# masnottuh/point-cloud-toolbox

Measured on AMD Instinct MI355X. Metric: points/sec curvature (1M-pt torus, k=50); HBM GB/s k-NN vs peak, higher is better.
Workload: dtype f64

## Files before the change

### point-cloud-toolbox_amd/csrc/pct_grid.hip

```cpp
#include "pct_internal.h"
#include "pct_grid_edge.h"

#include <math.h>
#include <stdlib.h>

namespace {

constexpr int kBlock = 256;

__device__ __forceinline__ float wave_min(float v) {
    for (int o = 32; o > 0; o >>= 1) v = fminf(v, __shfl_xor(v, o));
    return v;
}
__device__ __forceinline__ float wave_max(float v) {
    for (int o = 32; o > 0; o >>= 1) v = fmaxf(v, __shfl_xor(v, o));
    return v;
}

struct PackRed {
    int bb[6];
    int bad;
    int g_begin;
    double s[3], ss[3];
    unsigned long long cnt;
// ... 441 lines not shown
        }
        rank_of[i] = atomicAdd(&cell_oth[c], 1) | (int)0x80000000;
    }
}

__global__ __launch_bounds__(kBlock) void k_hist_raw(const float* __restrict__ xyz, int64_t n, pct_grid g, int q_begin, int q_end,
                                                     int* __restrict__ cell_of, int* __restrict__ rank_of,
                                                     int* __restrict__ cell_own, int* __restrict__ cell_oth, PackRed* __restrict__ parts) {
    const float sh[3] = {0.f, 0.f, 0.f};
    PackAcc acc;
    acc.init();
    const int64_t i = (int64_t)blockIdx.x * kBlock + threadIdx.x;
    if (i < n) {
        const float x = xyz[3 * i + 0], y = xyz[3 * i + 1], z = xyz[3 * i + 2];
        const bool ok = isfinite(x) && isfinite(y) && isfinite(z);
        acc.bad |= !ok;
        if (ok) acc.add(x, y, z, sh);
        const int cx = cell_coord(ok ? (double)x : g.ox, g.ox, g.inv_cell, g.nx);
        const int cy = cell_coord(ok ? (double)y : g.oy, g.oy, g.inv_cell, g.ny);
        const int cz = cell_coord(ok ? (double)z : g.oz, g.oz, g.inv_cell, g.nz);
        const int c = (cz * g.ny + cy) * g.nx + cx;
        cell_of[i] = c;
        if (i >= q_begin && i < q_end) rank_of[i] = atomicAdd(&cell_own[c], 1);
        else rank_of[i] = atomicAdd(&cell_oth[c], 1) | (int)0x80000000;
    }
    if (parts) acc.commit(parts + blockIdx.x);
}

__global__ __launch_bounds__(kBlock) void k_hist_agg(const float4* __restrict__ pts4, int64_t n, pct_grid g,
                                                     const float* __restrict__ own_want, float own_lo, float own_hi, int skip_outside,
                                                     int* __restrict__ cell_of, int* __restrict__ rank_of,
                                                     int* __restrict__ cell_own, int* __restrict__ cell_oth) {
    const int64_t i = (int64_t)blockIdx.x * kBlock + threadIdx.x;
    const int lane = threadIdx.x & 63;
    int key = -1;
    if (i < n) {
        const float4 p = pts4[i];
        bool inside = true;
        if (skip_outside) {
            const double fx = floor(((double)p.x - g.ox) * g.inv_cell), fy = floor(((double)p.y - g.oy) * g.inv_cell),
                         fz = floor(((double)p.z - g.oz) * g.inv_cell);
            inside = !(fx < 0 || fx >= g.nx || fy < 0 || fy >= g.ny || fz < 0 || fz >= g.nz);
        }
        if (inside) {
            const int cx = cell_coord((double)p.x, g.ox, g.inv_cell, g.nx);
            const int cy = cell_coord((double)p.y, g.oy, g.inv_cell, g.ny);
            const int cz = cell_coord((double)p.z, g.oz, g.inv_cell, g.nz);
            const int c = (cz * g.ny + cy) * g.nx + cx;
            const float w = own_want[__float_as_int(p.w)];
            const bool owned = w >= own_lo && w < own_hi;
            if (owned || !skip_outside || __builtin_nontemporal_load(&cell_oth[c]) <= 2048) key = 2 * c + (owned ? 1 : 0);
        }
    }
    int rank = 0;
    unsigned long long todo = __builtin_amdgcn_ballot_w64(key >= 0);
    while (todo) {
        const int leader = (int)__builtin_ctzll(todo);
        const int k0 = __builtin_amdgcn_readlane(key, leader);
        const unsigned long long same = __builtin_amdgcn_ballot_w64(key == k0);
        int base = 0;
        if (lane == leader) base = atomicAdd((k0 & 1) ? &cell_own[k0 >> 1] : &cell_oth[k0 >> 1], (int)__popcll(same));
        base = __builtin_amdgcn_readlane(base, leader);
        if (key == k0) rank = base + (int)__popcll(same & ((1ull << lane) - 1ull));
        todo &= ~same;
    }
    if (i < n) {
        cell_of[i] = key < 0 ? -1 : key >> 1;
        if (key >= 0) rank_of[i] = (key & 1) ? rank : (rank | (int)0x80000000);
    }
}

constexpr int kScanItems = 8;
constexpr int kScanTile = kBlock * kScanItems;

__device__ __forceinline__ int4 add3(int4 a, int4 b) { return make_int4(a.x + b.x, a.y + b.y, a.z + b.z, a.w + b.w); }

__device__ __forceinline__ int4 cell_counts(const int* __restrict__ own, const int* __restrict__ oth, int64_t c, int64_t ncell, int items_q) {
    if (c >= ncell) return make_int4(0, 0, 0, 0);
    const int o = own[c];
    const int t = o + (oth ? oth[c] : 0);
    return make_int4(t, (o + items_q - 1) / items_q, o, t > 0 ? 1 : 0);
}

__global__ __launch_bounds__(kBlock) void k_scan_sums(const int* __restrict__ own, const int* __restrict__ oth, int64_t ncell, int items_q,
                                                      int4* __restrict__ tmp, unsigned long long* __restrict__ sq_part) {
    __shared__ int4 sh[kBlock / 64];
    __shared__ unsigned long long shq[kBlock / 64];
    unsigned long long sq = 0;
    int64_t base = (int64_t)blockIdx.x * kScanTile + (int64_t)threadIdx.x * kScanItems;
    int4 v = make_int4(0, 0, 0, 0);
    for (int j = 0; j < kScanItems; ++j) {
        const int4 x = cell_counts(own, oth, base + j, ncell, items_q);
        v = add3(v, x);
        sq += (unsigned long long)x.z * (unsigned)x.x;
    }
    for (int o = 32; o > 0; o >>= 1) {
        v.x += __shfl_xor(v.x, o); v.y += __shfl_xor(v.y, o); v.z += __shfl_xor(v.z, o); v.w += __shfl_xor(v.w, o);
        sq += __shfl_xor(sq, o);
    }
    if ((threadIdx.x & 63) == 0) {
        sh[threadIdx.x >> 6] = v;
        shq[threadIdx.x >> 6] = sq;
    }
    __syncthreads();
    if (threadIdx.x == 0) {
        int4 t = make_int4(0, 0, 0, 0);
        unsigned long long q = 0;
        for (int i = 0; i < kBlock / 64; ++i) { t = add3(t, sh[i]); q += shq[i]; }
        tmp[blockIdx.x] = t;
        sq_part[blockIdx.x] = q;
    }
}

struct ScanTotals { unsigned long long sumsq; int4 tot; };

__global__ __launch_bounds__(1024) void k_scan_tiles(int4* __restrict__ tmp, int nblk, const unsigned long long* __restrict__ sq_part,
                                                      ScanTotals* __restrict__ host_copy, unsigned long long* __restrict__ zero8) {
    __shared__ int4 sh[1024];
    if (zero8 && threadIdx.x < 8) zero8[threadIdx.x] = 0ull;
    __shared__ int4 carry;
    __shared__ unsigned long long shq[16];
    {
        unsigned long long q = 0;
        for (int i = threadIdx.x; i < nblk; i += 1024) q += sq_part[i];
        for (int o = 32; o > 0; o >>= 1) q += __shfl_xor(q, o);
        if ((threadIdx.x & 63) == 0) shq[threadIdx.x >> 6] = q;
        __syncthreads();
        if (threadIdx.x == 0) { unsigned long long t = 0; for (int i = 0; i < 16; ++i) t += shq[i]; host_copy->sumsq = t; }
    }
    if (threadIdx.x == 0) carry = make_int4(0, 0, 0, 0);
    __syncthreads();
    for (int base = 0; base < nblk; base += 1024) {
        int i = base + threadIdx.x;
        int4 v = i < nblk ? tmp[i] : make_int4(0, 0, 0, 0);
        sh[threadIdx.x] = v;
        __syncthreads();
        for (int o = 1; o < 1024; o <<= 1) {
            int4 a = make_int4(0, 0, 0, 0);
            if ((int)threadIdx.x >= o) a = sh[threadIdx.x - o];
            __syncthreads();
            sh[threadIdx.x] = add3(sh[threadIdx.x], a);
            __syncthreads();
        }
        int4 incl = sh[threadIdx.x];
        int4 c = carry;
        if (i < nblk) tmp[i] = make_int4(c.x + incl.x - v.x, c.y + incl.y - v.y, c.z + incl.z - v.z, 0);
        __syncthreads();
        if (threadIdx.x == 1023) carry = add3(c, incl);
        __syncthreads();
    }
    if (threadIdx.x == 0) { tmp[nblk] = carry; host_copy->tot = carry; }
}

__global__ __launch_bounds__(kBlock) void k_scan_apply(const int* __restrict__ own, const int* __restrict__ oth, int64_t ncell, int items_q,
                                                       const int4* __restrict__ tmp, int* __restrict__ cell_start,
                                                       int* __restrict__ own_start, int2* __restrict__ items) {
    __shared__ int4 sh[kBlock];
    int64_t base = (int64_t)blockIdx.x * kScanTile + (int64_t)threadIdx.x * kScanItems;
    int4 x[kScanItems];
    int4 v = make_int4(0, 0, 0, 0);
    for (int j = 0; j < kScanItems; ++j) {
        x[j] = cell_counts(own, oth, base + j, ncell, items_q);
        v = add3(v, x[j]);
    }
    sh[threadIdx.x] = v;
    __syncthreads();
// ... 111 lines not shown
                const bool ok = isfinite(p[j].x) && isfinite(p[j].y) && isfinite(p[j].z);
                acc.bad |= !ok;
                if (ok) acc.add(p[j].x, p[j].y, p[j].z, sh);
            }
            atomicAdd(&s_cnt[bin_cell(p[j].x, p[j].y, p[j].z, g) >> shift], 1u);
        }
    }
    __syncthreads();
    for (int b = threadIdx.x; b < nb; b += kBinWide) mat[(size_t)blockIdx.x * nb + b] = s_cnt[b];
    if (parts) acc.commit<kBinWide / 64>(parts + blockIdx.x);
}

constexpr int kBinScanCols = 16, kBinScanGroups = 64, kBinScanPer = kBinMaxTiles / kBinScanGroups;
__global__ __launch_bounds__(kBinScanCols * kBinScanGroups) void k_bin_colscan(unsigned* __restrict__ mat, int ntiles, int nb, unsigned* __restrict__ tot) {
    __shared__ unsigned s[kBinScanGroups][kBinScanCols];
    const int lane = threadIdx.x % kBinScanCols, grp = threadIdx.x / kBinScanCols;
    const int col = blockIdx.x * kBinScanCols + lane;
    const int per = (ntiles + kBinScanGroups - 1) / kBinScanGroups;
    const int t0 = grp * per;
    unsigned v[kBinScanPer], sum = 0;
#pragma unroll
    for (int j = 0; j < kBinScanPer; ++j) {
        v[j] = (j < per && t0 + j < ntiles && col < nb) ? mat[(size_t)(t0 + j) * nb + col] : 0u;
        sum += v[j];
    }
    s[grp][lane] = sum;
    __syncthreads();
    unsigned run = 0;
    for (int q = 0; q < grp; ++q) run += s[q][lane];
    if (col >= nb) return;
#pragma unroll
    for (int j = 0; j < kBinScanPer; ++j) {
        if (j < per && t0 + j < ntiles) mat[(size_t)(t0 + j) * nb + col] = run;
        run += v[j];
    }
    if (grp == kBinScanGroups - 1) tot[col] = run;
}

__global__ __launch_bounds__(1024) void k_bin_plan(const unsigned* __restrict__ tot, int nb, int chunk, int* __restrict__ plan,
                                                   int4* __restrict__ items) {
    __shared__ int4 sh[1024];
    constexpr int per = kBinMaxBuckets / 1024;
    int4 v[per];
    int4 mine = make_int4(0, 0, 0, 0);
    for (int j = 0; j < per; ++j) {
        const int b = threadIdx.x * per + j;
        const int c = b < nb ? (int)tot[b] : 0;
        const int ni = b < nb ? max(1, (c + chunk - 1) / chunk) : 0;
        v[j] = make_int4(c, ni, ni > 1 ? ni : 0, ni > 1 ? 1 : 0);
        mine = add3(mine, v[j]);
    }
    sh[threadIdx.x] = mine;
    __syncthreads();
    for (int o = 1; o < 1024; o <<= 1) {
        int4 a = make_int4(0, 0, 0, 0);
        if ((int)threadIdx.x >= o) a = sh[threadIdx.x - o];
        __syncthreads();
        sh[threadIdx.x] = add3(sh[threadIdx.x], a);
        __syncthreads();
    }
    int4 run = make_int4(sh[threadIdx.x].x - mine.x, sh[threadIdx.x].y - mine.y, sh[threadIdx.x].z - mine.z, 0);
    int* bstart = plan + 16;
    for (int j = 0; j < per; ++j) {
        const int b = threadIdx.x * per + j;
        if (b < nb) {
            bstart[b] = run.x;
            for (int ch = 0; ch < v[j].y; ++ch)
                items[run.y + ch] = make_int4(b, run.x + ch * chunk, run.x + min(v[j].x, (ch + 1) * chunk), v[j].z ? run.z + ch : -1);
        }
        run = add3(run, v[j]);
    }
    if (threadIdx.x == 1023) {
        bstart[nb] = run.x;
        plan[0] = run.y;
        plan[1] = run.z;
        plan[2] = sh[1023].w;
    }
}

template <bool RAW>
__global__ __launch_bounds__(kBinWide) void k_bin_scatter(const float* __restrict__ xyz, const float4* __restrict__ pts4, int64_t n,
                                                           int tile_rows, pct_grid g, int shift, int nb, int chunk,
                                                           const unsigned* __restrict__ mat, const int* __restrict__ plan,
                                                           float4* __restrict__ rec, int* __restrict__ cell_own, int* __restrict__ cell_oth) {
    __shared__ unsigned s_cur[kBinMaxBuckets];
    const int* bstart = plan + 16;
    for (int b = threadIdx.x; b < nb; b += kBinWide) s_cur[b] = (unsigned)bstart[b] + mat[(size_t)blockIdx.x * nb + b];
    __syncthreads();
    const int64_t r0 = (int64_t)blockIdx.x * tile_rows, r1 = min(n, r0 + tile_rows);
    for (int64_t base = r0 + threadIdx.x; base < r1; base += 4 * kBinWide) {
        float4 p[4];
#pragma unroll
        for (int j = 0; j < 4; ++j)
            if (base + j * kBinWide < r1) p[j] = bin_load<RAW>(xyz, pts4, base + j * kBinWide);
#pragma unroll
        for (int j = 0; j < 4; ++j) {
            if (base + j * kBinWide >= r1) continue;
            const unsigned pos = atomicAdd(&s_cur[bin_cell(p[j].x, p[j].y, p[j].z, g) >> shift], 1u);
            if (pos < (unsigned)n) rec[pos] = p[j];
        }
    }
    if (plan[2] > 0) {
        for (int b = blockIdx.x; b < nb; b += gridDim.x) {
            if (bstart[b + 1] - bstart[b] <= chunk) continue;
            const int64_t c0 = (int64_t)b << shift, c1 = min(g.ncell, c0 + ((int64_t)1 << shift));
            for (int64_t c = c0 + threadIdx.x; c < c1; c += kBinWide) {
                cell_own[c] = 0;
                if (cell_oth) cell_oth[c] = 0;
            }
        }
    }
}

__global__ __launch_bounds__(kBinBlock) void k_bin_cells(const float4* __restrict__ rec, const int* __restrict__ plan,
                                                         const int4* __restrict__ items, pct_grid g, int shift, int q_begin, int q_end,
                                                         int* __restrict__ cell_own, int* __restrict__ cell_oth, int* __restrict__ base,
                                                         const PackRed* __restrict__ parts, int n_parts, PackRed* __restrict__ red,
                                                         PackRed* __restrict__ red_host) {
    extern __shared__ int s_c[];
    if (blockIdx.x == gridDim.x - 1) {
        if (parts) pack_fold<kBinBlock>(parts, n_parts, red, red_host, 0);
        return;
    }
    if ((int)blockIdx.x >= plan[0]) return;
    const int4 it = items[blockIdx.x];
    const int r0 = it.y, r1 = it.z, slot = it.w;
    const int cpb = 1 << shift, nc = cell_oth ? 2 * cpb : cpb;
    const int64_t c0 = (int64_t)it.x << shift;
    const int ncl = (int)min((int64_t)cpb, g.ncell - c0);
    for (int k = threadIdx.x; k < nc; k += kBinBlock) s_c[k] = 0;
    __syncthreads();
    for (int base = r0 + threadIdx.x; base < r1; base += 4 * kBinBlock) {
        float4 p[4];
#pragma unroll
        for (int j = 0; j < 4; ++j)
            if (base + j * kBinBlock < r1) p[j] = rec[base + j * kBinBlock];
#pragma unroll
        for (int j = 0; j < 4; ++j) {
            if (base + j * kBinBlock >= r1) continue;
            const int l = bin_cell(p[j].x, p[j].y, p[j].z, g) - (int)c0;
            const int idx = __float_as_int(p[j].w);
            const bool owned = !cell_oth || (idx >= q_begin && idx < q_end);
            if ((unsigned)l < (unsigned)cpb) atomicAdd(&s_c[(owned ? 0 : cpb) + l], 1);
        }
    }
    __syncthreads();
    for (int k = threadIdx.x; k < nc; k += kBinBlock) {
        const int l = k & (cpb - 1);
        if (l >= ncl) continue;
        int* arr = k < cpb ? cell_own : cell_oth;
        const int v = s_c[k];
        if (slot < 0) arr[c0 + l] = v;
        else base[(size_t)slot * nc + k] = v ? atomicAdd(&arr[c0 + l], v) : 0;
    }
}

__global__ __launch_bounds__(kBinBlock) void k_bin_place(const float4* __restrict__ rec, const int* __restrict__ plan,
                                                         const int4* __restrict__ items, pct_grid g, int shift, int q_begin, int q_end,
                                                         int64_t n, int64_t n_owned, const int* __restrict__ cell_start,
                                                         const int* __restrict__ cell_own, const int* __restrict__ cell_oth,
                                                         const int* __restrict__ own_start, const int* __restrict__ base,
                                                         float4* __restrict__ sorted4, int* __restrict__ row_of, int* __restrict__ owned_pos,
                                                         const double4* __restrict__ pts4d, double4* __restrict__ sorted4d) {
    extern __shared__ int s_cur[];
    if ((int)blockIdx.x >= plan[0]) return;
    const int4 it = items[blockIdx.x];
    const int r0 = it.y, r1 = it.z, slot = it.w;
    if (r0 >= r1) return;
    const int cpb = 1 << shift, nc = cell_oth ? 2 * cpb : cpb;
    const int64_t c0 = (int64_t)it.x << shift;
    const int ncl = (int)min((int64_t)cpb, g.ncell - c0);
    int* s_row = s_cur + nc;
    for (int k = threadIdx.x; k < nc; k += kBinBlock) {
        const int l = k & (cpb - 1);
        if (l >= ncl) continue;
        int s = cell_start[c0 + l];
        if (k >= cpb) s += cell_own[c0 + l];
        else if (cell_oth) s_row[l] = own_start[c0 + l] - s;
        if (slot >= 0) s += base[(size_t)slot * nc + k];
        s_cur[k] = s;
    }
    __syncthreads();
    for (int base = r0 + threadIdx.x; base < r1; base += 4 * kBinBlock) {
        float4 p[4];
#pragma unroll
        for (int j = 0; j < 4; ++j)
            if (base + j * kBinBlock < r1) p[j] = rec[base + j * kBinBlock];
#pragma unroll
        for (int j = 0; j < 4; ++j) {
            if (base + j * kBinBlock >= r1) continue;
            const int l = bin_cell(p[j].x, p[j].y, p[j].z, g) - (int)c0;
            const int idx = __float_as_int(p[j].w);
            const bool owned = !cell_oth || (idx >= q_begin && idx < q_end);
            if ((unsigned)l >= (unsigned)ncl) continue;
            const int pos = atomicAdd(&s_cur[(owned ? 0 : cpb) + l], 1);
            if ((unsigned)pos >= (unsigned)n) continue;
            sorted4[pos] = p[j];
            if (pts4d) sorted4d[pos] = pts4d[idx];
            if (owned) {
                const int row = cell_oth ? pos + s_row[l] : pos;
                if ((unsigned)row < (unsigned)n_owned && (unsigned)(idx - q_begin) < (unsigned)n_owned) {
                    owned_pos[row] = pos;
                    if (row_of) row_of[idx - q_begin] = row;
                }
            }
        }
    }
}

__global__ __launch_bounds__(256) void k_bin_row_of(const float4* __restrict__ sorted4, const int* __restrict__ owned_pos, int64_t n_owned,
                                                    int q_begin, int* __restrict__ row_of) {
    const int64_t row = (int64_t)blockIdx.x * 256 + threadIdx.x;
    if (row >= n_owned) return;
    const int idx = __float_as_int(sorted4[owned_pos[row]].w);
    if ((unsigned)(idx - q_begin) < (unsigned)n_owned) row_of[idx - q_begin] = (int)row;
}

__global__ __launch_bounds__(256) void k_gather_int(const int* __restrict__ map, int* __restrict__ io, int64_t n) {
    const int64_t i = (int64_t)blockIdx.x * 256 + threadIdx.x;
    if (i < n) io[i] = map[io[i]];
}

int grid_1d(int64_t n, int per_block, int cap) {
    int64_t b = (n + per_block - 1) / per_block;
    if (b < 1) b = 1;
    if (cap > 0 && b > cap) b = cap;
    return (int)b;
}

}

static PackRed* red_parts(pct_ctx* ctx) { return (PackRed*)((char*)ctx->red.p + 128); }
static_assert(sizeof(PackRed) <= sizeof(pct_pinned::pack_red) && alignof(PackRed) <= 128, "pct_pinned::pack_red holds a PackRed");
static_assert(sizeof(ScanTotals) <= sizeof(pct_pinned::scan_totals) && alignof(ScanTotals) <= 128, "pct_pinned::scan_totals holds a ScanTotals");
static PackRed* pin_red(pct_ctx* ctx) { return (PackRed*)ctx->pin->pack_red; }
static ScanTotals* pin_totals(pct_ctx* ctx) { return (ScanTotals*)ctx->pin->scan_totals; }

static int red_reset(pct_ctx* ctx, int n_parts, bool zero = true) {
    PCT_TRY(pct_reserve(ctx, &ctx->red, 128 + (size_t)n_parts * sizeof(PackRed)));
    if (zero) PCT_HIP(ctx, hipMemsetAsync(ctx->red.p, 0, 128, ctx->stream));
    return PCT_OK;
}

static int red_fold(pct_ctx* ctx, int n_parts, bool carry = true) {
    PCT_LAUNCH(k_pack_final, dim3(1), dim3(kBlock), 0, ctx->stream, (const PackRed*)red_parts(ctx), n_parts,
                       (PackRed*)ctx->red.p, pin_red(ctx), carry ? 1 : 0);
    PCT_HIP(ctx, hipGetLastError());
    return PCT_OK;
}

static int red_read(pct_ctx* ctx, int n_parts, PackRed* out, float* bbox, bool carry = true) {
    PCT_TRY(red_fold(ctx, n_parts, carry));
    PCT_HIP(ctx, hipStreamSynchronize(ctx->stream));
    memcpy(out, pin_red(ctx), sizeof(*out));
    for (int a = 0; a < 6; ++a) bbox[a] = order_float(out->bb[a]);
    return PCT_OK;
}

static int pack_all(pct_ctx* ctx, float* bbox, PackRed* red, bool defer = false, unsigned long long* begin_stamp = nullptr) {
    const int64_t n = ctx->n;
    PCT_TRY(pct_reserve(ctx, &ctx->pts4, (size_t)n * sizeof(float4)));
    const int nb = grid_1d(n, kBlock * 4, 512);
    PCT_TRY(red_reset(ctx, nb, false));
    PCT_LAUNCH(k_pack, dim3(nb), dim3(kBlock), 0, ctx->stream, ctx->xyz_view, n, (float4*)ctx->pts4.p, red_parts(ctx), begin_stamp);
    PCT_HIP(ctx, hipGetLastError());
    if (defer) {
        PCT_TRY(red_fold(ctx, nb, false));
    } else {
        PCT_TRY(red_read(ctx, nb, red, bbox, false));
        if (red->bad) return pct_fail(ctx, PCT_ERR_NONFINITE, "Non-finite values in input points");
// ... 244 lines not shown
        break;
    }
    s->raw = s->deferred_box = s->src == GridSource::CallerRows;
    s->from_base = s->src == GridSource::LevelBase;
    s->n = ctx->n_grid;
    s->g_begin = own_flag ? 0 : (int)ctx->g_begin;
    s->g_end = own_flag ? 0 : (int)(ctx->g_begin + n_owned);
    return PCT_OK;
}

enum class BoxCheck { Accept, Restart, NonFinite };
static BoxCheck check_deferred_box(pct_ctx* ctx, GridPoints* s) {
    s->deferred_box = false;
    memcpy(&s->red, pin_red(ctx), sizeof(s->red));
    if (s->red.bad) return BoxCheck::NonFinite;
    bool same = true;
    for (int ax = 0; ax < 3; ++ax) {
        const float lo = order_float(s->red.bb[ax]), hi = order_float(s->red.bb[3 + ax]);
        const float tol = 0.02f * (ctx->spec_raw[3 + ax] - ctx->spec_raw[ax]) + 1e-30f;
        same = same && fabsf(lo - ctx->spec_raw[ax]) <= tol && fabsf(hi - ctx->spec_raw[3 + ax]) <= tol;
    }
    return same ? BoxCheck::Accept : BoxCheck::Restart;
}

static void size_grid(const pct_ctx* ctx, bool sub_box, float* bbox, double a, pct_grid* g) {
    if (sub_box)
        for (int ax = 0; ax < 3; ++ax) {
            bbox[ax] = ctx->level_box[ax] - (float)(2.5 * a);
            bbox[3 + ax] = ctx->level_box[3 + ax] + (float)(2.5 * a);
        }
    g->ox = bbox[0]; g->oy = bbox[1]; g->oz = bbox[2];
    g->cell = a;
    g->inv_cell = 1.0 / a;
    double ex = (double)bbox[3] - bbox[0], ey = (double)bbox[4] - bbox[1], ez = (double)bbox[5] - bbox[2];
    if (!(ex >= 0)) ex = 0;
    if (!(ey >= 0)) ey = 0;
    if (!(ez >= 0)) ez = 0;
    const double dx = floor(ex * g->inv_cell) + 1, dy = floor(ey * g->inv_cell) + 1, dz = floor(ez * g->inv_cell) + 1;
    if (!(dx * dy * dz < 4.0e18) || !(dx < 2.0e9) || !(dy < 2.0e9) || !(dz < 2.0e9)) {
        g->nx = g->ny = g->nz = 1 << 30;
        g->ncell = (int64_t)1 << 62;
        return;
    }
    g->nx = (int32_t)dx;
    g->ny = (int32_t)dy;
    g->nz = (int32_t)dz;
    g->ncell = (int64_t)g->nx * g->ny * g->nz;
}

static int reserve_lists(pct_ctx* ctx, int64_t n, int64_t n_owned) {
    PCT_TRY(pct_reserve(ctx, &ctx->cell_of, (size_t)n * sizeof(int)));
    PCT_TRY(pct_reserve(ctx, &ctx->cell_fill, (size_t)n * sizeof(int)));
    PCT_TRY(pct_reserve(ctx, &ctx->sorted4, (size_t)n * sizeof(float4)));
    PCT_TRY(pct_reserve(ctx, &ctx->row_of, (size_t)((ctx->own_flag ? n : n_owned) + 1) * sizeof(int)));
    PCT_TRY(pct_reserve(ctx, &ctx->owned_pos, (size_t)n_owned * sizeof(int)));
    if (ctx->has_f64) PCT_TRY(pct_reserve(ctx, &ctx->sorted4d, (size_t)n * sizeof(double4)));
    return PCT_OK;
}

static EdgeSearch edge_search(const pct_ctx* ctx, const GridPoints& s, double target, double eps) {
    EdgeSearch es = {};
    es.target = target; es.n = s.n; es.eps = eps;
    es.ex = (double)s.bbox[3] - s.bbox[0]; es.ey = (double)s.bbox[4] - s.bbox[1]; es.ez = (double)s.bbox[5] - s.bbox[2];
    es.hint_edge = ctx->hint_edge; es.hint_guess = ctx->hint_guess; es.hint_target = ctx->hint_target;
    es.level_edge = ctx->level_edge;
    es.max_iter = es.level_edge > 0 ? 1 : ctx->level_mode ? 2 : 8;
    return es;
}

enum class GridBuild {
    Bin,
    AtomicRaw,
    AtomicBase,
    AtomicPacked,
};
static GridBuild choose_build(bool bin_allowed, const BinShape& bs, const GridPoints& s) {
    return bin_allowed && bs.ok ? GridBuild::Bin : s.raw ? GridBuild::AtomicRaw : s.from_base ? GridBuild::AtomicBase : GridBuild::AtomicPacked;
}

struct BinScratch {
    int* plan;
    unsigned* tot;
    int4* items;
    size_t lds;
};
static int bin_scratch(pct_ctx* ctx, const BinShape& bs, int64_t n, BinScratch* b) {
    PCT_TRY(pct_reserve(ctx, &ctx->bin_rec, (size_t)n * sizeof(float4)));
    PCT_TRY(pct_reserve(ctx, &ctx->bin_mat, (size_t)bs.ntiles * bs.nb * sizeof(unsigned)));
    const size_t plan_words = 16 + (size_t)(bs.nb + 1) + (size_t)bs.nb;
    const size_t items_at = (plan_words * sizeof(int) + 15) / 16 * 16;
    PCT_TRY(pct_reserve(ctx, &ctx->bin_plan, items_at + (size_t)bs.max_items * sizeof(int4)));
    PCT_TRY(pct_reserve(ctx, &ctx->bin_base, (size_t)bs.max_shared * (bs.cls << bs.shift) * sizeof(int)));
    b->plan = (int*)ctx->bin_plan.p;
    b->tot = (unsigned*)(b->plan + 16 + bs.nb + 1);
    b->items = (int4*)((char*)ctx->bin_plan.p + items_at);
    b->lds = (size_t)(bs.cls << bs.shift) * sizeof(int);
    return PCT_OK;
}

struct GridPass {
    GridBuild build;
    pct_grid g;
    BinShape bs;
    BinScratch bin;
    const float4* src;
    int64_t n_owned;
    bool sharded, sub_box;
};

template <bool RAW>
static void launch_bin_count(pct_ctx* ctx, int64_t n, const GridPass& p, PackRed* parts, unsigned long long* begin_stamp) {
    PCT_LAUNCH_T(k_bin_count<RAW>, dim3(p.bs.ntiles), dim3(kBinWide), 0, ctx->stream, ctx->xyz_view, p.src, n, p.bs.tile_rows, p.g, p.bs.shift,
                 p.bs.nb, (unsigned*)ctx->bin_mat.p, parts, begin_stamp);
}
template <bool RAW>
static void launch_bin_scatter(pct_ctx* ctx, int64_t n, const GridPass& p, int* cell_oth) {
    PCT_LAUNCH_T(k_bin_scatter<RAW>, dim3(p.bs.ntiles), dim3(kBinWide), 0, ctx->stream, ctx->xyz_view, p.src, n, p.bs.tile_rows, p.g, p.bs.shift,
                 p.bs.nb, p.bs.chunk, (const unsigned*)ctx->bin_mat.p, (const int*)p.bin.plan, (float4*)ctx->bin_rec.p, (int*)ctx->cell_own.p, cell_oth);
}

static int launch_count(pct_ctx* ctx, const GridPoints& s, GridPass& p, pct_call_clock* clock) {
    const pct_grid& g = p.g;
    const int64_t n = s.n;
    const float* own_flag = (const float*)ctx->own_flag;
    const bool bin = p.build == GridBuild::Bin;
    PCT_TRY(pct_reserve(ctx, &ctx->cell_own, (size_t)g.ncell * sizeof(int)));
    if (clock && !bin) PCT_HIP(ctx, clock->begin_event(ctx->stream));
    if (!bin) PCT_HIP(ctx, hipMemsetAsync(ctx->cell_own.p, 0, (size_t)g.ncell * sizeof(int), ctx->stream));
    if (p.sharded) {
        PCT_TRY(pct_reserve(ctx, &ctx->cell_oth, (size_t)g.ncell * sizeof(int)));
        if (!bin) PCT_HIP(ctx, hipMemsetAsync(ctx->cell_oth.p, 0, (size_t)g.ncell * sizeof(int), ctx->stream));
    }
    if (bin) PCT_TRY(bin_scratch(ctx, p.bs, n, &p.bin));
    int* cell_oth = p.sharded ? (int*)ctx->cell_oth.p : nullptr;
    PackRed* parts = s.deferred_box ? red_parts(ctx) : nullptr;
    const int nhb = grid_1d(n, kBlock, 0);
    if (bin) {
        const BinShape& bs = p.bs;
        unsigned long long* begin_stamp = clock ? clock->begin_word() : nullptr;
        s.raw ? launch_bin_count<true>(ctx, n, p, parts, begin_stamp) : launch_bin_count<false>(ctx, n, p, parts, begin_stamp);
        PCT_LAUNCH(k_bin_colscan, dim3((bs.nb + kBinScanCols - 1) / kBinScanCols), dim3(kBinScanCols * kBinScanGroups), 0, ctx->stream,
                   (unsigned*)ctx->bin_mat.p, bs.ntiles, bs.nb, p.bin.tot);
        PCT_LAUNCH(k_bin_plan, dim3(1), dim3(1024), 0, ctx->stream, (const unsigned*)p.bin.tot, bs.nb, bs.chunk, p.bin.plan, p.bin.items);
        s.raw ? launch_bin_scatter<true>(ctx, n, p, cell_oth) : launch_bin_scatter<false>(ctx, n, p, cell_oth);
        PCT_LAUNCH(k_bin_cells, dim3(bs.max_items + 1), dim3(kBinBlock), p.bin.lds, ctx->stream, (const float4*)ctx->bin_rec.p, (const int*)p.bin.plan,
                   (const int4*)p.bin.items, g, bs.shift, (int)ctx->q_begin, (int)ctx->q_end, (int*)ctx->cell_own.p, cell_oth,
                   (int*)ctx->bin_base.p, (const PackRed*)parts, bs.ntiles, (PackRed*)ctx->red.p, pin_red(ctx));
    } else if (p.build == GridBuild::AtomicRaw) {
        PCT_LAUNCH(k_hist_raw, dim3(nhb), dim3(kBlock), 0, ctx->stream, ctx->xyz_view, n, g, s.g_begin, s.g_end, (int*)ctx->cell_of.p,
                   (int*)ctx->cell_fill.p, (int*)ctx->cell_own.p, cell_oth, parts);
        if (parts) PCT_TRY(red_fold(ctx, nhb, false));
    } else if (p.build == GridBuild::AtomicBase) {
        PCT_LAUNCH(k_hist_agg, dim3(nhb), dim3(kBlock), 0, ctx->stream, p.src, n, g, own_flag, ctx->own_lo, ctx->own_hi, p.sub_box ? 1 : 0,
                   (int*)ctx->cell_of.p, (int*)ctx->cell_fill.p, (int*)ctx->cell_own.p, (int*)ctx->cell_oth.p);
    } else {
        PCT_LAUNCH(k_hist, dim3(nhb), dim3(kBlock), 0, ctx->stream, p.src, n, g, s.g_begin, s.g_end, own_flag, ctx->own_lo, ctx->own_hi,
                   p.sub_box ? 1 : 0, (int*)ctx->cell_of.p, (int*)ctx->cell_fill.p, (int*)ctx->cell_own.p, cell_oth);
    }
    return PCT_OK;
}

static int launch_scan(pct_ctx* ctx, const GridPass& p, int items_q, int nblk) {
    const int* cell_oth = p.sharded ? (const int*)ctx->cell_oth.p : nullptr;
    PCT_TRY(pct_reserve(ctx, &ctx->scan_tmp, (size_t)(nblk + 1) * sizeof(int4) + (size_t)nblk * sizeof(unsigned long long)));
    unsigned long long* sq_part = (unsigned long long*)((int4*)ctx->scan_tmp.p + nblk + 1);
    PCT_TRY(pct_reserve(ctx, &ctx->cell_cnt, (size_t)(p.g.ncell + 1) * sizeof(int)));
    PCT_TRY(pct_reserve(ctx, &ctx->own_start, (size_t)(p.g.ncell + 1) * sizeof(int)));
    PCT_TRY(pct_reserve(ctx, &ctx->occ, ((size_t)(p.n_owned < p.g.ncell ? p.n_owned : p.g.ncell) + (size_t)p.n_owned / items_q + 16) * sizeof(int2)));
    PCT_LAUNCH(k_scan_sums, dim3(nblk), dim3(kBlock), 0, ctx->stream, (const int*)ctx->cell_own.p, cell_oth, p.g.ncell, items_q,
               (int4*)ctx->scan_tmp.p, sq_part);
    PCT_TRY(pct_reserve(ctx, &ctx->counters, sizeof(pct_dev_words)));
    PCT_LAUNCH(k_scan_tiles, dim3(1), dim3(1024), 0, ctx->stream, (int4*)ctx->scan_tmp.p, nblk,
               (const unsigned long long*)sq_part, pin_totals(ctx), (unsigned long long*)&pct_dev(ctx)->sweep);
    ctx->counters_clean = true;
    PCT_HIP(ctx, hipEventRecord(ctx->ev[PCT_EV_SCAN_TOTALS], ctx->stream));
    PCT_LAUNCH(k_scan_apply, dim3(nblk), dim3(kBlock), 0, ctx->stream, (const int*)ctx->cell_own.p, cell_oth, p.g.ncell, items_q,
               (const int4*)ctx->scan_tmp.p, (int*)ctx->cell_cnt.p, (int*)ctx->own_start.p, (int2*)ctx->occ.p);
    return PCT_OK;
}

static int launch_place(pct_ctx* ctx, const GridPoints& s, const GridPass& p) {
    const pct_grid& g = p.g;
    const int64_t n = s.n;
    const bool lazy_rows = p.build == GridBuild::Bin && !ctx->level_mode;
    ctx->row_of_valid = !lazy_rows;
    ctx->row_of_rows = p.n_owned;
    ctx->row_of_begin = (int)ctx->q_begin;
    const int* cell_oth = p.sharded ? (const int*)ctx->cell_oth.p : nullptr;
    const double4* pts4d = ctx->has_f64 ? (const double4*)ctx->pts4d.p : nullptr;
    double4* sorted4d = ctx->has_f64 ? (double4*)ctx->sorted4d.p : nullptr;
    if (p.build == GridBuild::Bin)
        PCT_LAUNCH(k_bin_place, dim3(p.bs.max_items), dim3(kBinBlock), p.bin.lds + (p.sharded ? p.bin.lds / 2 : 0), ctx->stream,
                   (const float4*)ctx->bin_rec.p, (const int*)p.bin.plan, (const int4*)p.bin.items, g, p.bs.shift, (int)ctx->q_begin,
                   (int)ctx->q_end, n, p.n_owned, (const int*)ctx->cell_cnt.p, (const int*)ctx->cell_own.p, cell_oth,
                   (const int*)ctx->own_start.p, (const int*)ctx->bin_base.p, (float4*)ctx->sorted4.p,
                   lazy_rows ? nullptr : (int*)ctx->row_of.p, (int*)ctx->owned_pos.p, pts4d, sorted4d);
    else if (p.build == GridBuild::AtomicRaw)
        PCT_LAUNCH(k_scatter_raw, dim3(grid_1d(n, kBlock, 0)), dim3(kBlock), 0, ctx->stream, ctx->xyz_view, (const int*)ctx->cell_of.p,
                   (const int*)ctx->cell_cnt.p, (const int*)ctx->cell_own.p, (const int*)ctx->own_start.p, (const int*)ctx->cell_fill.p, n,
                   s.g_begin, (float4*)ctx->sorted4.p, (int*)ctx->row_of.p, (int*)ctx->owned_pos.p, pts4d, sorted4d);
    else
        PCT_LAUNCH(k_scatter, dim3(grid_1d(n, kBlock, 0)), dim3(kBlock), 0, ctx->stream, p.src, (const int*)ctx->cell_of.p,
                   (const int*)ctx->cell_cnt.p, (const int*)ctx->cell_own.p, (const int*)ctx->own_start.p, (const int*)ctx->cell_fill.p, n,
                   s.g_begin, (float4*)ctx->sorted4.p, (int*)ctx->row_of.p, (int*)ctx->owned_pos.p, pts4d, sorted4d);
    PCT_HIP(ctx, hipGetLastError());
    return PCT_OK;
}

static int debug_bin_plan(pct_ctx* ctx, const GridPass& p) {
    int pw[3] = {0, 0, 0};
    PCT_HIP(ctx, hipMemcpyAsync(pw, p.bin.plan, sizeof(pw), hipMemcpyDeviceToHost, ctx->stream));
    PCT_HIP(ctx, hipStreamSynchronize(ctx->stream));
    fprintf(stderr, "[grid] bin build: %d buckets of %d cells, %d tiles of %d rows, %d work items of up to %d records, %d of them in %d shared buckets\n",
            p.bs.nb, 1 << p.bs.shift, p.bs.ntiles, p.bs.tile_rows, pw[0], p.bs.chunk, pw[1], pw[2]);
    return PCT_OK;
}

static int commit_grid(pct_ctx* ctx, const GridPoints& s, pct_grid g, const EdgeSearch& es, int iters, double m_last, int4 tot,
                       int64_t n_owned, bool sub_box) {
    const bool own_flag = ctx->own_flag != nullptr, level_pass = es.level_edge > 0;
    const int64_t n = s.n;
    for (int ax = 0; ax < 3; ++ax) {
        const double o = ax == 0 ? g.ox : ax == 1 ? g.oy : g.oz;
        g.lim_lo[ax] = ctx->culled ? ((double)s.kept_box.lo[ax] - o) * g.inv_cell : -INFINITY;
        g.lim_hi[ax] = ctx->culled ? ((double)s.kept_box.hi[ax] - o) * g.inv_cell : INFINITY;
    }
    if (pct_getenv("PCT_GRID_DEBUG"))
        fprintf(stderr, "[grid] box [%g %g %g]-[%g %g %g] edge %g dims %d x %d x %d = %lld cells, %d passes, occupancy %.1f, items %d\n", s.bbox[0],
                s.bbox[1], s.bbox[2], s.bbox[3], s.bbox[4], s.bbox[5], g.cell, g.nx, g.ny, g.nz, (long long)g.ncell, iters, m_last, tot.y);
    if (ctx->level_mode && !own_flag)
        for (int a = 0; a < 6; ++a) ctx->lvl_bbox[a] = s.bbox[a];
    ctx->grid = g;
    ctx->tm.grid_iters += iters;
    ctx->tm.cells = g.ncell;
    ctx->tm.cell_size = g.cell;
    ctx->tm.grid_points = n;
    ctx->tm.occupancy = m_last;
    if (s.src != GridSource::CulledPack && !own_flag && !ctx->level_mode) {
        for (int a = 0; a < 6; ++a) ctx->spec_bbox[a] = s.bbox[a];
        if (s.red.cnt > 0)
            for (int a = 0; a < 6; ++a) ctx->spec_raw[a] = order_float(s.red.bb[a]);
        ctx->spec_n = ctx->n;
        ctx->spec_valid = true;
    }
    if (m_last > 0 && !level_pass) {
        ctx->hint_edge = es.hint_after(g.cell, m_last);
        ctx->hint_guess = es.first_guess;
        ctx->hint_target = es.target;
    }
    if ((tot.x != n && !sub_box) || tot.x > n || tot.z != n_owned)
        return pct_fail(ctx, PCT_ERR_INVALID, "cell scan totals %d/%d != %lld/%lld", tot.x, tot.z, (long long)n, (long long)n_owned);
    if (!level_pass && m_last > 64.0 * es.target && m_last * 27.0 * (double)n_owned > 1e12)
        return pct_fail(ctx, PCT_ERR_INVALID,
                        "the cell list cannot resolve this cloud: a point shares its cell with %.0f others on average at the "
                        "smallest usable cell edge %.3g (%lld cells); thin it out or split it into compact pieces",
                        m_last, g.cell, (long long)g.ncell);
    ctx->n_items = tot.y;
    ctx->nonempty_cells = tot.w;
    ctx->n_occ = tot.y;
    ctx->tm.occupied_cells = tot.y;
    ctx->grid_valid = true;
    ctx->grid_whole = !own_flag && !ctx->level_mode && !sub_box && !ctx->culled && n == ctx->n && ctx->q_begin == 0 && ctx->q_end == ctx->n &&
                      ctx->slab_parts == 0;
    return PCT_OK;
}

int pct_build_grid(pct_ctx* ctx, int32_t k, double eps, bool may_give_up, GridVerdict* out, pct_call_clock* clock) {
    *out = GridVerdict::Built;
    ctx->grid_valid = false;
    const double factor = ctx->occupancy_factor > 0 ? ctx->occupancy_factor : pct_default_factor(k);
    const double target = factor * (k + 1);
    int64_t cell_cap = (int64_t)1 << 27;
    if (ctx->level_mode) cell_cap = (int64_t)1 << 24;
    else if (32 * ctx->n > cell_cap) cell_cap = 32 * ctx->n < ((int64_t)1 << 30) ? 32 * ctx->n : (int64_t)1 << 30;
    const bool own_flag = ctx->own_flag != nullptr;
    const bool slab = ctx->slab_parts >= 1 && !own_flag;
    const bool sub_box = ctx->level_edge > 0 && ctx->level_box_valid;
    const bool bin_allowed = !own_flag && !sub_box && !slab && !pct_getenv("PCT_GRID_ATOMIC");
    int items_q = 16;
    if (const char* e = pct_getenv("PCT_ITEMS_Q")) { const int v = atoi(e); if (v >= 1 && v <= 64) items_q = v; }

    for (int attempt = 0; attempt < 3; ++attempt) {
        ctx->tm.grid_iters = 0;
        if (slab) PCT_TRY(slab_split(ctx));
        const int64_t n_owned = own_flag ? ctx->own_count : ctx->q_end - ctx->q_begin;
        const bool sharded = own_flag || ctx->q_begin > 0 || ctx->q_end < ctx->n || slab;
        GridPoints s;
        bool restart = false;
        PCT_TRY(select_source(ctx, k, target, slab, n_owned, sharded, &s, &restart, clock));
        if (restart) continue;
        const int64_t n = s.n;
        ctx->items_q = items_q;
        PCT_TRY(reserve_lists(ctx, n, n_owned));
        EdgeSearch es = edge_search(ctx, s, target, eps);
        double a = es.first();
        GridPass p = {};
        p.src = s.from_base ? (const float4*)ctx->lvl_src.p : (const float4*)ctx->pts4.p;
        p.n_owned = n_owned; p.sharded = sharded; p.sub_box = sub_box;
        int iters = 0;
        int4 tot = make_int4(0, 0, 0, 0);
        double m_last = 0;
        for (int it = 0; it < es.max_iter; ++it) {
            a = es.clamp_eps(a);
            size_grid(ctx, sub_box, s.bbox, a, &p.g);
            if (!own_flag && !(es.level_edge > 0) && p.g.ncell > 16 * n && p.g.ncell > ((int64_t)1 << 20)) {
                if (it == 0 && es.hinted) {
                    a = es.fallback_first();
                    size_grid(ctx, sub_box, s.bbox, a, &p.g);
                } else if (may_give_up) {
                    *out = GridVerdict::GaveUp;
                    ctx->grid_valid = false;
                    return PCT_OK;
                }
            }
            bool hit_cap = false;
            while (p.g.ncell > cell_cap) {
                a *= cbrt((double)p.g.ncell / (double)cell_cap) * 1.01;
                size_grid(ctx, sub_box, s.bbox, a, &p.g);
                hit_cap = true;
            }
            const pct_grid& g = p.g;
            p.bs = bin_allowed ? bin_shape(n, g.ncell, sharded) : BinShape{};
            p.build = choose_build(bin_allowed, p.bs, s);
            const bool bin = p.build == GridBuild::Bin;
            PCT_TRY(launch_count(ctx, s, p, clock));
            const int nblk = (int)((g.ncell + kScanTile - 1) / kScanTile);
            if (pct_getenv("PCT_GRID_DEBUG"))
                fprintf(stderr, "[grid] pass %d: n %lld owned %lld edge %g dims %d x %d x %d = %lld cells (%d scan tiles), box [%g %g %g]-[%g %g %g]\n", it,
                        (long long)n, (long long)n_owned, a, g.nx, g.ny, g.nz, (long long)g.ncell, nblk, s.bbox[0], s.bbox[1], s.bbox[2], s.bbox[3], s.bbox[4], s.bbox[5]);
            PCT_TRY(launch_scan(ctx, p, items_q, nblk));
            PCT_TRY(launch_place(ctx, s, p));
            PCT_HIP(ctx, hipEventSynchronize(ctx->ev[PCT_EV_SCAN_TOTALS]));
            if (s.deferred_box) {
                const BoxCheck box = check_deferred_box(ctx, &s);
                if (box == BoxCheck::NonFinite) return pct_fail(ctx, PCT_ERR_NONFINITE, "Non-finite values in input points");
                if (box == BoxCheck::Restart) {
                    ctx->spec_valid = false;
                    restart = true;
                    break;
                }
            }
            if (bin && pct_getenv("PCT_GRID_DEBUG")) PCT_TRY(debug_bin_plan(ctx, p));
            tot = pin_totals(ctx)->tot;
            m_last = (double)pin_totals(ctx)->sumsq / (double)(n_owned > 0 ? n_owned : 1);
            ++iters;
            if (es.accept(m_last, a, g.ncell, cell_cap, hit_cap, it)) break;
            a = es.next(m_last, a);
        }
        if (restart) continue;
        return commit_grid(ctx, s, p.g, es, iters, m_last, tot, n_owned, sub_box);
    }
    return pct_fail(ctx, PCT_ERR_INVALID, "cell-list build: restarted more than twice");
}

int pct_ensure_row_of(pct_ctx* ctx) {
    if (ctx->row_of_valid) return PCT_OK;
    const int64_t rows = ctx->row_of_rows;
    if (rows > 0) {
        PCT_LAUNCH(k_bin_row_of, dim3((unsigned)((rows + 255) / 256)), dim3(256), 0, ctx->stream, (const float4*)ctx->sorted4.p,
                   (const int*)ctx->owned_pos.p, rows, ctx->row_of_begin, (int*)ctx->row_of.p);
        PCT_HIP(ctx, hipGetLastError());
    }
    ctx->row_of_valid = true;
    return PCT_OK;
}

int pct_launch_gather_int(pct_ctx* ctx, const int* d_map, int* d_inout, int64_t n) {
    PCT_LAUNCH(k_gather_int, dim3((unsigned)((n + 255) / 256)), dim3(256), 0, ctx->stream, d_map, d_inout, n);
    PCT_HIP(ctx, hipGetLastError());
    return PCT_OK;
}
```

Measured before the change: 1.563 billion.

## Fuse cell-count scan into bin kernels, dropping scan_sums and scan_apply passes

In the binned grid build path, k_bin_cells now has the last item block of each bucket, picked through an atomic ticket, compute per-bucket scan totals (counts, items, owned, occupancy, sum of squares). k_bin_place does the per-cell exclusive scan locally with DPP wave prefix sums and writes cell_start, own_start and occ itself. This removes the separate k_scan_sums and k_scan_apply launches and their extra passes over the cell arrays. The cost is ticket atomics with acquire fences and more work in the place kernel, and the cross-block ordering makes the code more fragile.

```diff
diff --git a/point-cloud-toolbox_amd/csrc/pct_grid.hip b/point-cloud-toolbox_amd/csrc/pct_grid.hip
--- a/point-cloud-toolbox_amd/csrc/pct_grid.hip
+++ b/point-cloud-toolbox_amd/csrc/pct_grid.hip
@@ -547,6 +547,11 @@
     return make_int4(t, (o + items_q - 1) / items_q, o, t > 0 ? 1 : 0);
 }
 
+__device__ __forceinline__ int4 count_record(int o, int x, int items_q) {
+    const int t = o + x;
+    return make_int4(t, (o + items_q - 1) / items_q, o, t > 0 ? 1 : 0);
+}
+
 __global__ __launch_bounds__(kBlock) void k_scan_sums(const int* __restrict__ own, const int* __restrict__ oth, int64_t ncell, int items_q,
                                                       int4* __restrict__ tmp, unsigned long long* __restrict__ sq_part) {
     __shared__ int4 sh[kBlock / 64];
@@ -824,7 +829,8 @@
 __global__ __launch_bounds__(kBinWide) void k_bin_scatter(const float* __restrict__ xyz, const float4* __restrict__ pts4, int64_t n,
                                                            int tile_rows, pct_grid g, int shift, int nb, int chunk,
                                                            const unsigned* __restrict__ mat, const int* __restrict__ plan,
-                                                           float4* __restrict__ rec, int* __restrict__ cell_own, int* __restrict__ cell_oth) {
+                                                           float4* __restrict__ rec, int* __restrict__ cell_own, int* __restrict__ cell_oth,
+                                                           unsigned* __restrict__ tickets) {
     __shared__ unsigned s_cur[kBinMaxBuckets];
     const int* bstart = plan + 16;
     for (int b = threadIdx.x; b < nb; b += kBinWide) s_cur[b] = (unsigned)bstart[b] + mat[(size_t)blockIdx.x * nb + b];
@@ -845,6 +851,7 @@
     if (plan[2] > 0) {
         for (int b = blockIdx.x; b < nb; b += gridDim.x) {
             if (bstart[b + 1] - bstart[b] <= chunk) continue;
+            if (threadIdx.x == 0) tickets[b] = 0u;
             const int64_t c0 = (int64_t)b << shift, c1 = min(g.ncell, c0 + ((int64_t)1 << shift));
             for (int64_t c = c0 + threadIdx.x; c < c1; c += kBinWide) {
                 cell_own[c] = 0;
@@ -854,12 +861,27 @@
     }
 }
 
+__device__ __forceinline__ int wave_incl_sum(int v) {
+    v += __builtin_amdgcn_update_dpp(0, v, 0x111, 0xf, 0xf, false);
+    v += __builtin_amdgcn_update_dpp(0, v, 0x112, 0xf, 0xf, false);
+    v += __builtin_amdgcn_update_dpp(0, v, 0x114, 0xf, 0xf, false);
+    v += __builtin_amdgcn_update_dpp(0, v, 0x118, 0xf, 0xf, false);
+    v += __builtin_amdgcn_update_dpp(0, v, 0x142, 0xa, 0xf, false);
+    v += __builtin_amdgcn_update_dpp(0, v, 0x143, 0xc, 0xf, false);
+    return v;
+}
+
 __global__ __launch_bounds__(kBinBlock) void k_bin_cells(const float4* __restrict__ rec, const int* __restrict__ plan,
                                                          const int4* __restrict__ items, pct_grid g, int shift, int q_begin, int q_end,
                                                          int* __restrict__ cell_own, int* __restrict__ cell_oth, int* __restrict__ base,
                                                          const PackRed* __restrict__ parts, int n_parts, PackRed* __restrict__ red,
-                                                         PackRed* __restrict__ red_host) {
+                                                         PackRed* __restrict__ red_host, int items_q, int chunk,
+                                                         int4* __restrict__ brec, unsigned long long* __restrict__ bsq,
+                                                         unsigned* __restrict__ tickets) {
     extern __shared__ int s_c[];
+    __shared__ int4 s_rec[kBinBlock / 64];
+    __shared__ unsigned long long s_sq[kBinBlock / 64];
+    __shared__ int s_last;
     if (blockIdx.x == gridDim.x - 1) {
         if (parts) pack_fold<kBinBlock>(parts, n_parts, red, red_host, 0);
         return;
@@ -895,39 +917,123 @@
         if (slot < 0) arr[c0 + l] = v;
         else base[(size_t)slot * nc + k] = v ? atomicAdd(&arr[c0 + l], v) : 0;
     }
+    if (slot >= 0) {
+        __syncthreads();
+        if (threadIdx.x == 0) {
+            const int* bstart = plan + 16;
+            const int ni = (bstart[it.x + 1] - bstart[it.x] + chunk - 1) / chunk;
+            const bool last = atomicAdd(&tickets[it.x], 1u) == (unsigned)(ni - 1);
+            if (last) __builtin_amdgcn_fence(__ATOMIC_ACQUIRE, "agent");
+            s_last = last;
+        }
+        __syncthreads();
+        if (!s_last) return;
+    }
+    int4 v = make_int4(0, 0, 0, 0);
+    unsigned long long sq = 0;
+    for (int l = threadIdx.x; l < ncl; l += kBinBlock) {
+        int o, x = 0;
+        if (slot < 0) {
+            o = s_c[l];
+            if (cell_oth) x = s_c[cpb + l];
+        } else {
+            o = __hip_atomic_load(&cell_own[c0 + l], __ATOMIC_RELAXED, __HIP_MEMORY_SCOPE_AGENT);
+            if (cell_oth) x = __hip_atomic_load(&cell_oth[c0 + l], __ATOMIC_RELAXED, __HIP_MEMORY_SCOPE_AGENT);
+        }
+        const int4 c = count_record(o, x, items_q);
+        v = add3(v, c);
+        sq += (unsigned long long)c.z * (unsigned)c.x;
+    }
+    v = make_int4(wave_incl_sum(v.x), wave_incl_sum(v.y), wave_incl_sum(v.z), wave_incl_sum(v.w));
+    for (int o = 32; o > 0; o >>= 1) sq += __shfl_xor(sq, o);
+    if ((threadIdx.x & 63) == 63) {
+        s_rec[threadIdx.x >> 6] = v;
+        s_sq[threadIdx.x >> 6] = sq;
+    }
+    __syncthreads();
+    if (threadIdx.x == 0) {
+        int4 t = make_int4(0, 0, 0, 0);
+        unsigned long long q = 0;
+        for (int i = 0; i < kBinBlock / 64; ++i) { t = add3(t, s_rec[i]); q += s_sq[i]; }
+        brec[it.x] = t;
+        bsq[it.x] = q;
+    }
 }
 
 __global__ __launch_bounds__(kBinBlock) void k_bin_place(const float4* __restrict__ rec, const int* __restrict__ plan,
                                                          const int4* __restrict__ items, pct_grid g, int shift, int q_begin, int q_end,
-                                                         int64_t n, int64_t n_owned, const int* __restrict__ cell_start,
+                                                         int64_t n, int64_t n_owned, int nb, int items_q, const int4* __restrict__ brec,
                                                          const int* __restrict__ cell_own, const int* __restrict__ cell_oth,
-                                                         const int* __restrict__ own_start, const int* __restrict__ base,
+                                                         const int* __restrict__ base, int* __restrict__ cell_start,
+                                                         int* __restrict__ own_start, int2* __restrict__ occ, int64_t occ_cap,
                                                          float4* __restrict__ sorted4, int* __restrict__ row_of, int* __restrict__ owned_pos,
                                                          const double4* __restrict__ pts4d, double4* __restrict__ sorted4d) {
     extern __shared__ int s_cur[];
+    __shared__ int4 s_wave[kBinBlock / 64];
     if ((int)blockIdx.x >= plan[0]) return;
     const int4 it = items[blockIdx.x];
     const int r0 = it.y, r1 = it.z, slot = it.w;
-    if (r0 >= r1) return;
     const int cpb = 1 << shift, nc = cell_oth ? 2 * cpb : cpb;
     const int64_t c0 = (int64_t)it.x << shift;
     const int ncl = (int)min((int64_t)cpb, g.ncell - c0);
     int* s_row = s_cur + nc;
-    for (int k = threadIdx.x; k < nc; k += kBinBlock) {
-        const int l = k & (cpb - 1);
+    float4 p[4];
+#pragma unroll
+    for (int j = 0; j < 4; ++j)
+        if (r0 + (int)threadIdx.x + j * kBinBlock < r1) p[j] = rec[r0 + threadIdx.x + j * kBinBlock];
+    const int lane = threadIdx.x & 63, wave = threadIdx.x >> 6;
+    const int l_begin = wave * (cpb / (kBinBlock / 64)), l_end = l_begin + cpb / (kBinBlock / 64);
+    {
+        int4 v = make_int4(0, 0, 0, 0);
+        for (int l = l_begin + lane; l < l_end; l += 64) {
+            const int o = l < ncl ? cell_own[c0 + l] : 0, x = cell_oth && l < ncl ? cell_oth[c0 + l] : 0;
+            s_cur[l] = o;
+            if (cell_oth) s_cur[cpb + l] = x;
+            v = add3(v, count_record(o, x, items_q));
+        }
+        v = make_int4(wave_incl_sum(v.x), wave_incl_sum(v.y), wave_incl_sum(v.z), 0);
+        if (lane == 63) s_wave[wave] = v;
+    }
+    __syncthreads();
+    int4 run = brec[it.x];
+    for (int w = 0; w < wave; ++w) run = add3(run, s_wave[w]);
+    const bool first = slot < 0 || r0 == plan[16 + it.x];
+    for (int l = l_begin + lane; l < l_end; l += 64) {
+        const int o = s_cur[l], x = cell_oth ? s_cur[cpb + l] : 0;
+        const int4 c = count_record(o, x, items_q);
+        const int4 incl = make_int4(wave_incl_sum(c.x), wave_incl_sum(c.y), wave_incl_sum(c.z), 0);
+        const int s = run.x + incl.x - c.x, r = run.y + incl.y - c.y, w = run.z + incl.z - c.z;
+        run.x += __builtin_amdgcn_readlane(incl.x, 63);
+        run.y += __builtin_amdgcn_readlane(incl.y, 63);
+        run.z += __builtin_amdgcn_readlane(incl.z, 63);
         if (l >= ncl) continue;
-        int s = cell_start[c0 + l];
-        if (k >= cpb) s += cell_own[c0 + l];
-        else if (cell_oth) s_row[l] = own_start[c0 + l] - s;
-        if (slot >= 0) s += base[(size_t)slot * nc + k];
-        s_cur[k] = s;
-    }
+        const size_t off = slot >= 0 ? (size_t)slot * nc + l : 0;
+        const int run_own = slot >= 0 ? base[off] : 0, run_oth = slot >= 0 && cell_oth ? base[off + cpb] : 0;
+        if (first) {
+            cell_start[c0 + l] = s;
+            own_start[c0 + l] = w;
+            for (int ch = 0; ch < c.y; ++ch)
+                if (r + ch < occ_cap) occ[r + ch] = make_int2((int)(c0 + l), ch);
+        }
+        s_cur[l] = s + run_own;
+        if (cell_oth) {
+            s_cur[cpb + l] = s + o + run_oth;
+            s_row[l] = w - s;
+        }
+    }
+    if (first && it.x == nb - 1 && threadIdx.x == 0) {
+        const int4 tot = brec[nb];
+        cell_start[g.ncell] = tot.x;
+        own_start[g.ncell] = tot.z;
+    }
+    if (r0 >= r1) return;
     __syncthreads();
     for (int base = r0 + threadIdx.x; base < r1; base += 4 * kBinBlock) {
-        float4 p[4];
-#pragma unroll
-        for (int j = 0; j < 4; ++j)
-            if (base + j * kBinBlock < r1) p[j] = rec[base + j * kBinBlock];
+        if (base != r0 + (int)threadIdx.x) {
+#pragma unroll
+            for (int j = 0; j < 4; ++j)
+                if (base + j * kBinBlock < r1) p[j] = rec[base + j * kBinBlock];
+        }
 #pragma unroll
         for (int j = 0; j < 4; ++j) {
             if (base + j * kBinBlock >= r1) continue;
@@ -1338,6 +1444,9 @@
     int* plan;
     unsigned* tot;
     int4* items;
+    int4* brec;
+    unsigned long long* bsq;
+    unsigned* tickets;
     size_t lds;
 };
 static int bin_scratch(pct_ctx* ctx, const BinShape& bs, int64_t n, BinScratch* b) {
@@ -1345,11 +1454,17 @@
     PCT_TRY(pct_reserve(ctx, &ctx->bin_mat, (size_t)bs.ntiles * bs.nb * sizeof(unsigned)));
     const size_t plan_words = 16 + (size_t)(bs.nb + 1) + (size_t)bs.nb;
     const size_t items_at = (plan_words * sizeof(int) + 15) / 16 * 16;
-    PCT_TRY(pct_reserve(ctx, &ctx->bin_plan, items_at + (size_t)bs.max_items * sizeof(int4)));
+    const size_t brec_at = items_at + (size_t)bs.max_items * sizeof(int4);
+    const size_t bsq_at = brec_at + (size_t)(bs.nb + 1) * sizeof(int4);
+    const size_t tickets_at = bsq_at + (size_t)bs.nb * sizeof(unsigned long long);
+    PCT_TRY(pct_reserve(ctx, &ctx->bin_plan, tickets_at + (size_t)bs.nb * sizeof(unsigned)));
     PCT_TRY(pct_reserve(ctx, &ctx->bin_base, (size_t)bs.max_shared * (bs.cls << bs.shift) * sizeof(int)));
     b->plan = (int*)ctx->bin_plan.p;
     b->tot = (unsigned*)(b->plan + 16 + bs.nb + 1);
     b->items = (int4*)((char*)ctx->bin_plan.p + items_at);
+    b->brec = (int4*)((char*)ctx->bin_plan.p + brec_at);
+    b->bsq = (unsigned long long*)((char*)ctx->bin_plan.p + bsq_at);
+    b->tickets = (unsigned*)((char*)ctx->bin_plan.p + tickets_at);
     b->lds = (size_t)(bs.cls << bs.shift) * sizeof(int);
     return PCT_OK;
 }
@@ -1362,6 +1477,8 @@
     const float4* src;
     int64_t n_owned;
     bool sharded, sub_box;
+    int items_q;
+    int64_t occ_cap;
 };
 
 template <bool RAW>
@@ -1372,7 +1489,8 @@
 template <bool RAW>
 static void launch_bin_scatter(pct_ctx* ctx, int64_t n, const GridPass& p, int* cell_oth) {
     PCT_LAUNCH_T(k_bin_scatter<RAW>, dim3(p.bs.ntiles), dim3(kBinWide), 0, ctx->stream, ctx->xyz_view, p.src, n, p.bs.tile_rows, p.g, p.bs.shift,
-                 p.bs.nb, p.bs.chunk, (const unsigned*)ctx->bin_mat.p, (const int*)p.bin.plan, (float4*)ctx->bin_rec.p, (int*)ctx->cell_own.p, cell_oth);
+                 p.bs.nb, p.bs.chunk, (const unsigned*)ctx->bin_mat.p, (const int*)p.bin.plan, (float4*)ctx->bin_rec.p, (int*)ctx->cell_own.p, cell_oth,
+                 p.bin.tickets);
 }
 
 static int launch_count(pct_ctx* ctx, const GridPoints& s, GridPass& p, pct_call_clock* clock) {
@@ -1401,7 +1519,8 @@
         s.raw ? launch_bin_scatter<true>(ctx, n, p, cell_oth) : launch_bin_scatter<false>(ctx, n, p, cell_oth);
         PCT_LAUNCH(k_bin_cells, dim3(bs.max_items + 1), dim3(kBinBlock), p.bin.lds, ctx->stream, (const float4*)ctx->bin_rec.p, (const int*)p.bin.plan,
                    (const int4*)p.bin.items, g, bs.shift, (int)ctx->q_begin, (int)ctx->q_end, (int*)ctx->cell_own.p, cell_oth,
-                   (int*)ctx->bin_base.p, (const PackRed*)parts, bs.ntiles, (PackRed*)ctx->red.p, pin_red(ctx));
+                   (int*)ctx->bin_base.p, (const PackRed*)parts, bs.ntiles, (PackRed*)ctx->red.p, pin_red(ctx), p.items_q, bs.chunk,
+                   p.bin.brec, p.bin.bsq, p.bin.tickets);
     } else if (p.build == GridBuild::AtomicRaw) {
         PCT_LAUNCH(k_hist_raw, dim3(nhb), dim3(kBlock), 0, ctx->stream, ctx->xyz_view, n, g, s.g_begin, s.g_end, (int*)ctx->cell_of.p,
                    (int*)ctx->cell_fill.p, (int*)ctx->cell_own.p, cell_oth, parts);
@@ -1416,22 +1535,27 @@
     return PCT_OK;
 }
 
-static int launch_scan(pct_ctx* ctx, const GridPass& p, int items_q, int nblk) {
+static int launch_scan(pct_ctx* ctx, const GridPass& p, int nblk) {
+    const bool bin = p.build == GridBuild::Bin;
+    const int items_q = p.items_q;
     const int* cell_oth = p.sharded ? (const int*)ctx->cell_oth.p : nullptr;
-    PCT_TRY(pct_reserve(ctx, &ctx->scan_tmp, (size_t)(nblk + 1) * sizeof(int4) + (size_t)nblk * sizeof(unsigned long long)));
-    unsigned long long* sq_part = (unsigned long long*)((int4*)ctx->scan_tmp.p + nblk + 1);
+    if (!bin) PCT_TRY(pct_reserve(ctx, &ctx->scan_tmp, (size_t)(nblk + 1) * sizeof(int4) + (size_t)nblk * sizeof(unsigned long long)));
+    int4* tmp = bin ? p.bin.brec : (int4*)ctx->scan_tmp.p;
+    unsigned long long* sq_part = bin ? p.bin.bsq : (unsigned long long*)((int4*)ctx->scan_tmp.p + nblk + 1);
+    if (bin) nblk = p.bs.nb;
     PCT_TRY(pct_reserve(ctx, &ctx->cell_cnt, (size_t)(p.g.ncell + 1) * sizeof(int)));
     PCT_TRY(pct_reserve(ctx, &ctx->own_start, (size_t)(p.g.ncell + 1) * sizeof(int)));
-    PCT_TRY(pct_reserve(ctx, &ctx->occ, ((size_t)(p.n_owned < p.g.ncell ? p.n_owned : p.g.ncell) + (size_t)p.n_owned / items_q + 16) * sizeof(int2)));
-    PCT_LAUNCH(k_scan_sums, dim3(nblk), dim3(kBlock), 0, ctx->stream, (const int*)ctx->cell_own.p, cell_oth, p.g.ncell, items_q,
-               (int4*)ctx->scan_tmp.p, sq_part);
+    PCT_TRY(pct_reserve(ctx, &ctx->occ, (size_t)p.occ_cap * sizeof(int2)));
+    if (!bin)
+        PCT_LAUNCH(k_scan_sums, dim3(nblk), dim3(kBlock), 0, ctx->stream, (const int*)ctx->cell_own.p, cell_oth, p.g.ncell, items_q, tmp, sq_part);
     PCT_TRY(pct_reserve(ctx, &ctx->counters, sizeof(pct_dev_words)));
-    PCT_LAUNCH(k_scan_tiles, dim3(1), dim3(1024), 0, ctx->stream, (int4*)ctx->scan_tmp.p, nblk,
+    PCT_LAUNCH(k_scan_tiles, dim3(1), dim3(1024), 0, ctx->stream, tmp, nblk,
                (const unsigned long long*)sq_part, pin_totals(ctx), (unsigned long long*)&pct_dev(ctx)->sweep);
     ctx->counters_clean = true;
     PCT_HIP(ctx, hipEventRecord(ctx->ev[PCT_EV_SCAN_TOTALS], ctx->stream));
-    PCT_LAUNCH(k_scan_apply, dim3(nblk), dim3(kBlock), 0, ctx->stream, (const int*)ctx->cell_own.p, cell_oth, p.g.ncell, items_q,
-               (const int4*)ctx->scan_tmp.p, (int*)ctx->cell_cnt.p, (int*)ctx->own_start.p, (int2*)ctx->occ.p);
+    if (!bin)
+        PCT_LAUNCH(k_scan_apply, dim3(nblk), dim3(kBlock), 0, ctx->stream, (const int*)ctx->cell_own.p, cell_oth, p.g.ncell, items_q,
+                   (const int4*)tmp, (int*)ctx->cell_cnt.p, (int*)ctx->own_start.p, (int2*)ctx->occ.p);
     return PCT_OK;
 }
 
@@ -1448,8 +1572,9 @@
     if (p.build == GridBuild::Bin)
         PCT_LAUNCH(k_bin_place, dim3(p.bs.max_items), dim3(kBinBlock), p.bin.lds + (p.sharded ? p.bin.lds / 2 : 0), ctx->stream,
                    (const float4*)ctx->bin_rec.p, (const int*)p.bin.plan, (const int4*)p.bin.items, g, p.bs.shift, (int)ctx->q_begin,
-                   (int)ctx->q_end, n, p.n_owned, (const int*)ctx->cell_cnt.p, (const int*)ctx->cell_own.p, cell_oth,
-                   (const int*)ctx->own_start.p, (const int*)ctx->bin_base.p, (float4*)ctx->sorted4.p,
+                   (int)ctx->q_end, n, p.n_owned, p.bs.nb, p.items_q, (const int4*)p.bin.brec, (const int*)ctx->cell_own.p, cell_oth,
+                   (const int*)ctx->bin_base.p, (int*)ctx->cell_cnt.p, (int*)ctx->own_start.p, (int2*)ctx->occ.p, p.occ_cap,
+                   (float4*)ctx->sorted4.p,
                    lazy_rows ? nullptr : (int*)ctx->row_of.p, (int*)ctx->owned_pos.p, pts4d, sorted4d);
     else if (p.build == GridBuild::AtomicRaw)
         PCT_LAUNCH(k_scatter_raw, dim3(grid_1d(n, kBlock, 0)), dim3(kBlock), 0, ctx->stream, ctx->xyz_view, (const int*)ctx->cell_of.p,
@@ -1552,7 +1677,7 @@
         double a = es.first();
         GridPass p = {};
         p.src = s.from_base ? (const float4*)ctx->lvl_src.p : (const float4*)ctx->pts4.p;
-        p.n_owned = n_owned; p.sharded = sharded; p.sub_box = sub_box;
+        p.n_owned = n_owned; p.sharded = sharded; p.sub_box = sub_box; p.items_q = items_q;
         int iters = 0;
         int4 tot = make_int4(0, 0, 0, 0);
         double m_last = 0;
@@ -1579,12 +1704,13 @@
             p.bs = bin_allowed ? bin_shape(n, g.ncell, sharded) : BinShape{};
             p.build = choose_build(bin_allowed, p.bs, s);
             const bool bin = p.build == GridBuild::Bin;
+            p.occ_cap = (n_owned < g.ncell ? n_owned : g.ncell) + n_owned / items_q + 16;
             PCT_TRY(launch_count(ctx, s, p, clock));
             const int nblk = (int)((g.ncell + kScanTile - 1) / kScanTile);
             if (pct_getenv("PCT_GRID_DEBUG"))
                 fprintf(stderr, "[grid] pass %d: n %lld owned %lld edge %g dims %d x %d x %d = %lld cells (%d scan tiles), box [%g %g %g]-[%g %g %g]\n", it,
                         (long long)n, (long long)n_owned, a, g.nx, g.ny, g.nz, (long long)g.ncell, nblk, s.bbox[0], s.bbox[1], s.bbox[2], s.bbox[3], s.bbox[4], s.bbox[5]);
-            PCT_TRY(launch_scan(ctx, p, items_q, nblk));
+            PCT_TRY(launch_scan(ctx, p, nblk));
             PCT_TRY(launch_place(ctx, s, p));
             PCT_HIP(ctx, hipEventSynchronize(ctx->ev[PCT_EV_SCAN_TOTALS]));
             if (s.deferred_box) {
```

Result: faster. 1.584 billion, median of 6 (+1.3%).
